# lambdaclass/simpleworks

Hardware: AMD Instinct MI355X
Metric: Marlin prove() constraints/sec at 2^20 R1CS; G1 MSM points/sec (higher is better)
Workload: dtype u32 limbs (384-bit Montgomery Fq for G1, 256-bit Fr); 1 GPU; marlin_prove: synthetic R1CS, 2^20 constraints = variables = non-zeros per matrix (|H| = |K| = 2^20), SRS + proving key device resident; per_gpu_units=1048576, multi_gpu=replicas (one proof per rank)

## Files before the change

simpleworks_amd/_lib.py:

```python
import ctypes
import json
import os

import numpy as np

_HERE = os.path.dirname(os.path.abspath(__file__))
LIB_PATH = os.environ.get("SWM_LIB_PATH") or os.path.join(_HERE, "libswmarlin.so")

_u64p = ctypes.POINTER(ctypes.c_uint64)
_u32p = ctypes.POINTER(ctypes.c_uint32)
_vp = ctypes.c_void_p
_sz = ctypes.c_size_t
_int = ctypes.c_int

ABI = {
    "swm_version": (_int, []),
    "swm_strerror": (ctypes.c_char_p, [_int]),
    "swm_init": (_int, [_int, ctypes.POINTER(_vp)]),
    "swm_destroy": (None, [_vp]),
    "swm_last_error": (ctypes.c_char_p, [_vp]),
    "swm_set_stream": (_int, [_vp, _vp]),
    "swm_set_msm_sharding": (_int, [_vp, ctypes.c_uint, ctypes.c_uint, _vp, _vp]),
    "swm_rccl_unique_id": (_int, [ctypes.c_void_p]),
    "swm_rccl_init": (_int, [_vp, ctypes.c_void_p, ctypes.c_uint, ctypes.c_uint]),
# ... 415 lines not shown
                    "swm_selftest_g1_codec")
        return out, bad.value

    FR29_OPS = {"mul": 0, "mul_c": 1, "normalize": 2, "cond_sub_2r": 3, "cond_sub_r": 4, "canonical_below_2r": 5,
                "canonical": 6, "sub": 7, "unpack": 8, "pack": 9, "inv": 10, "inv_exact": 11}

    def selftest_fr29(self, op, a9, b9=None, spread9=None):
        a = np.ascontiguousarray(a9, dtype=np.uint32).reshape(-1, 9)
        b = np.ascontiguousarray(b9 if b9 is not None else a, dtype=np.uint32).reshape(-1, 9)
        assert b.shape == a.shape
        sp = np.ascontiguousarray(spread9 if spread9 is not None else np.zeros(9), dtype=np.uint32).reshape(9)
        out = np.zeros_like(a)
        self._check(self.lib.swm_selftest_fr29(self.h, self.FR29_OPS[op], _p32(a), _p32(b), _p32(sp), _p32(out), a.shape[0]),
                    "swm_selftest_fr29")
        return out

    def _poly(self, op, data, n, m, z, pieces, out):
        zz = np.ascontiguousarray(z if z is not None else np.zeros(4), dtype=np.uint64).reshape(4)
        pc = np.ascontiguousarray(pieces if pieces is not None else np.zeros(2), dtype=np.uint64).reshape(-1)
        self._check(self.lib.swm_selftest_poly(self.h, op, data.ctypes.data, n, m, _p64(zz), _p64(pc), pc.size // 2,
                                               out.ctypes.data if out is not None else None), "swm_selftest_poly")

    def selftest_suffix_recurrence(self, a_mont, m, z_mont):
        a = np.ascontiguousarray(a_mont, dtype=np.uint64).reshape(-1, 4).copy()
        self._poly(0, a, a.shape[0], m, z_mont, None, None)
        return a

    def selftest_div_linear(self, p_mont, z_mont):
        p = np.ascontiguousarray(p_mont, dtype=np.uint64).reshape(-1, 4)
        out = np.zeros_like(p)
        self._poly(1, p, p.shape[0], 0, z_mont, None, out)
        return out

    def selftest_poly_eval(self, p_mont, z_mont):
        p = np.ascontiguousarray(p_mont, dtype=np.uint64).reshape(-1, 4)
        out = np.zeros(4, dtype=np.uint64)
        self._poly(2, p, p.shape[0], 0, z_mont, None, out)
        return out

    def selftest_poly_eval_many(self, buf_mont, pieces, z_mont):
        buf = np.ascontiguousarray(buf_mont, dtype=np.uint64).reshape(-1, 4)
        pc = np.asarray(pieces, dtype=np.uint64).reshape(-1, 2)
        out = np.zeros((pc.shape[0], 4), dtype=np.uint64)
        self._poly(3, buf, buf.shape[0], 0, z_mont, pc, out)
        return out

    def selftest_ntt_from(self, src_mont, log_n, inverse=False, coset=False):
        src = np.ascontiguousarray(src_mont, dtype=np.uint64).reshape(-1, 4).copy()
        out = np.zeros((1 << log_n, 4), dtype=np.uint64)
        self._poly(4 + int(bool(inverse)) + 2 * int(bool(coset)), src, src.shape[0], log_n, None, None, out)
        return out, src

    def selftest_ntt_cosets(self, coeffs_mont, log_n, ks):
        src = np.ascontiguousarray(coeffs_mont, dtype=np.uint64).reshape(-1, 4).copy()
        kk = np.ascontiguousarray(ks, dtype=np.uint64).reshape(-1)
        out = np.zeros((kk.size << log_n, 4), dtype=np.uint64)
        self._check(self.lib.swm_selftest_poly(self.h, 9, src.ctypes.data, src.shape[0], log_n, _p64(np.zeros(4, np.uint64)),
                                               _p64(kk), kk.size, out.ctypes.data), "swm_selftest_poly")
        return out.reshape(kk.size, 1 << log_n, 4)

    def selftest_intt_cosets3(self, evals_mont, log_n):
        ev = np.ascontiguousarray(evals_mont, dtype=np.uint64).reshape(-1, 4).copy()
        out = np.zeros_like(ev)
        self._poly(10, ev, ev.shape[0], log_n, None, None, out)
        return out

# ... 17 lines not shown
```

simpleworks_amd/csrc/devops.cuh:

```cuda
#pragma once
#include <chrono>
#include <exception>
#include <functional>
#include <utility>
#include <atomic>
#include "context.h"
#include "ff.cuh"
#include "fill.cuh"
#include "fr29.cuh"
#include "host/chacha.h"
#include "host/marlin_types.h"

namespace swm {

int ntt_run(swm_ctx* ctx, void* d_data, unsigned log_n, int inverse, int coset);
int ntt_run_from(swm_ctx* ctx, void* d_data, unsigned log_n, int inverse, int coset, const void* first_src, size_t src_len);
int ntt_cosets_fwd(swm_ctx* ctx, const void* coeffs, size_t len, unsigned log_n, const unsigned* ks, unsigned ncos, void* out);
int ntt_cosets_inv(swm_ctx* ctx, void* data, unsigned log_n, unsigned ncos);
int ntt_sharded_run(swm_ctx* ctx, void* d_local, unsigned log_n, int inverse, int blocks_in);
struct SpmvPlanHost {
    uint64_t nnz = 0, max_row = 0;
    std::vector<uint32_t> chunks, lrows;
};
struct SpmvPlan {
// ... 202 lines not shown

__device__ __forceinline__ Fr29 fr29_zero() {
    Fr29 r;
#pragma unroll
    for (int i = 0; i < 9; i++) r.l[i] = 0;
    return r;
}
__device__ __forceinline__ Fr29 fr29_below_2r(const Fr29& lazy_below_4r) {
    return fr29_cond_sub(fr29_normalize(lazy_below_4r), Fr29Consts::P2);
}
static __global__ void __launch_bounds__(256) rec_tile_total29(const Fr* __restrict__ a, size_t n, RecConsts rc,
                                                               const Fr* __restrict__ zlow ,
                                                               Fr* __restrict__ totals) {
    SWM_LIGHT_KERNEL();
    __shared__ Fr sm[256];
    const size_t base = (size_t)blockIdx.x * RT_TILE;
    const unsigned t = threadIdx.x;
    const Fr29 z256 = fr29_unpack(rc.z256);
    Fr29 acc = fr29_zero();
#pragma unroll 1
    for (int j = RT_PER - 1; j >= 0; j--) {
        size_t k = base + (size_t)j * 256 + t;
        acc = fr29_mul_fenced(acc, z256);
        if (k < n) acc = fr29_add(acc, fr29_unpack(a[k]));
    }
    sm[t] = fr29_pack(fr29_canonical(fr29_mul_fenced(acc, fr29_unpack(zlow[t])), true));
    __syncthreads();
    for (unsigned s = 128; s > 0; s >>= 1) {
        if (t < s) sm[t] = fp_add(sm[t], sm[t + s]);
        __syncthreads();
    }
    if (t == 0) totals[blockIdx.x] = fp_mul(sm[0], rc.zpow[0]);
}
static __global__ void __launch_bounds__(256) rec_tile_scan29(Fr* __restrict__ a, size_t n, RecConsts rc,
                                                              const Fr* __restrict__ tile_true , size_t ntiles) {
    SWM_LIGHT_KERNEL();
    extern __shared__ __align__(16) unsigned char smem_raw[];
    Fr* tile = reinterpret_cast<Fr*>(smem_raw);
    Fr* hs = tile + RT_TILE + 256;
    const size_t b = blockIdx.x, base = b * RT_TILE;
    const unsigned t = threadIdx.x;
#pragma unroll
    for (int j = 0; j < RT_PER; j++) {
        unsigned e = j * 256 + t;
        size_t k = base + e;
        tile[rt_pad(e)] = k < n ? a[k] : fp_zero<Fr>();
    }
    __syncthreads();
    Fr29 loc[RT_PER];
    {
        const Fr29 z1 = fr29_unpack(rc.zpow[1]);
        Fr29 acc = fr29_zero();
#pragma unroll
        for (int i = RT_PER - 1; i >= 0; i--) {
            acc = fr29_add(fr29_unpack(tile[rt_pad(t * RT_PER + i)]), fr29_mul_fenced(acc, z1));
            loc[i] = acc;
        }
        hs[t] = fr29_pack(fr29_below_2r(acc));
    }
    if (t == 0) hs[256] = b + 1 < ntiles ? tile_true[b + 1] : fp_zero<Fr>();
    __syncthreads();
#pragma unroll 1
    for (int k = 0; k < 9; k++) {
        unsigned d = 1u << k;
        Fr v = hs[t];
        bool has = t + d <= 256;
        Fr o = has ? hs[t + d] : fp_zero<Fr>();
        __syncthreads();
        if (has) hs[t] = fr29_pack(fr29_below_2r(fr29_add(fr29_unpack(v), fr29_mul_fenced(fr29_unpack(o), fr29_unpack(rc.zstep[k])))));
        __syncthreads();
    }
    const Fr29 carry = fr29_unpack(hs[t + 1]);
#pragma unroll
    for (int i = 0; i < RT_PER; i++) {
        const Fr29 v = fr29_add(loc[i], fr29_mul_fenced(carry, fr29_unpack(rc.zpow[RT_PER - i])));
        tile[rt_pad(t * RT_PER + i)] = fr29_pack(fr29_cond_sub(fr29_cond_sub(fr29_cond_sub(fr29_normalize(v), Fr29Consts::P2), Fr29Consts::P2), Fr29Consts::P));
    }
    __syncthreads();
#pragma unroll
    for (int j = 0; j < RT_PER; j++) {
        unsigned e = j * 256 + t;
        size_t k = base + e;
        if (k < n) a[k] = tile[rt_pad(e)];
    }
}

inline void suffix_recurrence(swm_ctx* ctx, Fr* a, size_t n, size_t m, const Fr& z);
inline void suffix_recurrence_tiled(swm_ctx* ctx, Fr* a, size_t n, const Fr& z) {
    size_t ntiles = (n + RT_TILE - 1) / RT_TILE;
    RecConsts rc;
    rc.zpow[0] = fp_one<Fr>();
    for (int i = 1; i <= RT_PER; i++) rc.zpow[i] = fp_mul(rc.zpow[i - 1], z);
    rc.zstep[0] = rc.zpow[RT_PER];
    for (int k = 1; k < 9; k++) rc.zstep[k] = fp_sqr(rc.zstep[k - 1]);
    DVec zlow(ctx, 256), totals(ctx, ntiles);
    rc.z256 = dv_pow256(ctx, z, zlow.p);
    RecConsts rc29;
    const Fr two5 = fp_from_u64<Fr>(32);
    for (int i = 0; i <= RT_PER; i++) rc29.zpow[i] = fp_mul(rc.zpow[i], two5);
    for (int k = 0; k < 9; k++) rc29.zstep[k] = fp_mul(rc.zstep[k], two5);
    rc29.z256 = fp_mul(rc.z256, two5);
    prof_begin(ctx, "rec_tile_total");
    hipLaunchKernelGGL(rec_tile_total29, dim3((unsigned)ntiles), dim3(256), 0, ctx->stream, (const Fr*)a, n, rc29, (const Fr*)zlow.p, totals.p);
    prof_end(ctx);
    hip_check(ctx, hipGetLastError(), "rec_tile_total");
    Fr ztile = rc.z256;
    for (int i = 0; i < 3; i++) ztile = fp_sqr(ztile);
    static_assert(RT_TILE == 2048, "tile exponent");
    suffix_recurrence(ctx, totals.p, ntiles, 1, ztile);
    size_t lds = (size_t)(RT_TILE + 256 + 257) * sizeof(Fr);
    static std::atomic<bool> attr_set[64];
    if (!attr_set[ctx->device & 63].load(std::memory_order_acquire)) {
        hip_check(ctx, hipFuncSetAttribute((const void*)rec_tile_scan29, hipFuncAttributeMaxDynamicSharedMemorySize, (int)lds), "attr");
        attr_set[ctx->device & 63].store(true, std::memory_order_release);
    }
    prof_begin(ctx, "rec_tile_scan");
    hipLaunchKernelGGL(rec_tile_scan29, dim3((unsigned)ntiles), dim3(256), lds, ctx->stream, a, n, rc29, (const Fr*)totals.p, ntiles);
    prof_end(ctx);
    hip_check(ctx, hipGetLastError(), "rec_tile_scan");
}

inline void suffix_recurrence(swm_ctx* ctx, Fr* a, size_t n, size_t m, const Fr& z) {
    if (n == 0) return;
    if (m == 1 && n >= 4 * (size_t)RT_TILE) {
        suffix_recurrence_tiled(ctx, a, n, z);
        return;
    }
    size_t rows = (n + m - 1) / m;
    if (rows <= REC_T) {
        prof_begin(ctx, "rec_serial");
        hipLaunchKernelGGL(rec_serial, dim3((unsigned)((m + 63) / 64)), dim3(64), 0, ctx->stream, a, n, m, z);
        prof_end(ctx);
        hip_check(ctx, hipGetLastError(), "rec_serial");
        return;
    }
    size_t nblk = (rows + REC_T - 1) / REC_T;
    DVec head(ctx, nblk * m);
    unsigned grid = (unsigned)((nblk * m + 255) / 256);
    prof_begin(ctx, "rec_local");
    hipLaunchKernelGGL(rec_local, dim3(grid), dim3(256), 0, ctx->stream, a, n, m, z, head.p, nblk);
    prof_end(ctx);
    hip_check(ctx, hipGetLastError(), "rec_local");
    Fr zt = z;
    for (int i = 0; i < 4; i++) zt = fp_sqr(zt);
    static_assert(REC_T == 16, "zt exponent");
    suffix_recurrence(ctx, head.p, nblk * m, m, zt);
    prof_begin(ctx, "rec_fix");
    hipLaunchKernelGGL(rec_fix, dim3(grid), dim3(256), 0, ctx->stream, a, n, m, z, head.p, nblk);
    prof_end(ctx);
    hip_check(ctx, hipGetLastError(), "rec_fix");
}

struct DivResult {
    DVec work;
};
inline DivResult div_linear(swm_ctx* ctx, const Fr* p, size_t n, const Fr& x, size_t cap = 0) {
    DivResult r;
    r.work = dv_copy_padded(ctx, p, n, std::max<size_t>({n, cap, 1}));
    if (n == 0) r.work.zero();
    suffix_recurrence(ctx, r.work.p, n, 1, x);
    return r;
}

static constexpr int EVAL_PER = 16;
static constexpr int EVAL_TILE = 256 * EVAL_PER;
static __global__ void __launch_bounds__(256) eval_chunks(const Fr* __restrict__ c, size_t n, Fr x256, const Fr* __restrict__ xpow,
                                                          Fr* __restrict__ out) {
    SWM_LIGHT_KERNEL();
    __shared__ Fr sm[256];
    const size_t base = (size_t)blockIdx.x * EVAL_TILE;
    const unsigned t = threadIdx.x;
    Fr acc = fp_zero<Fr>();
#pragma unroll 1
    for (int j = EVAL_PER - 1; j >= 0; j--) {
        size_t k = base + (size_t)j * 256 + t;
        acc = fp_mul(acc, x256);
        if (k < n) acc = fp_add(acc, c[k]);
    }
    sm[t] = fp_mul(acc, xpow[t]);
    __syncthreads();
    for (unsigned s = 128; s > 0; s >>= 1) {
        if (t < s) sm[t] = fp_add(sm[t], sm[t + s]);
        __syncthreads();
    }
    if (t == 0) out[blockIdx.x] = sm[0];
}
struct EvalPoint {
    DVec pw[3];
    Fr y256[3];
};
inline EvalPoint eval_point(swm_ctx* ctx, Fr x) {
    EvalPoint ep;
    for (int l = 0; l < 3; l++) {
        ep.pw[l] = DVec(ctx, 256);
// ... 460 lines not shown
```

simpleworks_amd/csrc/marlin.hip:

```cpp
#include <stdlib.h>
#include <string.h>
#include <algorithm>
#include <chrono>
#include <functional>
#include <memory>
#include "devops.cuh"
#include "g1.cuh"
#include "host/ahp.h"

#include "msm.h"
using namespace swm;

#define LAUNCHX(ctx, name, kernel, grid, block, shmem, ...)                         \
    do {                                                                            \
        prof_begin(ctx, name);                                                      \
        hipLaunchKernelGGL(kernel, grid, block, shmem, (ctx)->stream, __VA_ARGS__); \
        prof_end(ctx);                                                              \
        hip_check(ctx, hipGetLastError(), name);                                    \
    } while (0)

#include "host/pk_codec.h"
#include "host/host_handles.h"
struct swm_srs {
    ~swm_srs() {
// ... 1010 lines not shown
    Fr t = fp_add(fp_add(fp_mul(fp_mul(c.eta_a, x.av[i]), dbc), fp_mul(fp_mul(fp_mul(c.eta_b, x.bv[i]), da), dc)),
                  fp_mul(fp_mul(fp_mul(c.eta_c, x.cv[i]), da), db));
    Fr a_val = fp_mul(c.vhab, t);
    Fr b_val = fp_mul(da, dbc);
    return fp_sub(a_val, fp_mul(b_val, f));
}
struct ProveState {
    ChaChaRng& zk;
    PhaseTrace& tr;
    const ProveShape shape;
    const ShardPlan sp;
    const uint64_t H, K, X, Bsz, M;
    const unsigned logM;
    const size_t nvars, ninst;
    const size_t mask_len;
    const HDomain dh;
    const std::vector<Fr> public_input;
    FiatShamirRng fs;
    VerifierState st;
    Fr rho_w, rho_a, rho_b;
    int lane = 0;
    LPoly P_w, P_za, P_zb, P_mask, P_t, P_g1, P_h1, P_g2, P_h2;
    LPoly idx_polys[12];
    std::map<std::string, LPoly*> polys;
    CommitJob j1[4], j2[3], j3[2];
    std::vector<Commitment> comms1 = std::vector<Commitment>(4), comms2 = std::vector<Commitment>(3),
                            comms3 = std::vector<Commitment>(2);
    bool mask_late = false;
    unsigned mask_pieces = 1;
    AsyncMsm mask_part[2];
    bool ra_closed_form = false;
    bool cosets = false;
    LcSet lcs;
    DVec mask, z, za_evals, zb_evals, za_loc, zb_loc, x_poly, x_evals, w_poly, za_poly, zb_poly, e_za, e_zb, e_z;
    DVec r_alpha_evals, e_ra, t_poly, q1, h1, g1x, f, h2;

    ProveState(const swm_pk& pk, ChaChaRng& rng, PhaseTrace& t, ProveShape shp, const ShardPlan& plan)
        : zk(rng), tr(t), shape(std::move(shp)), sp(plan), H(pk.H), K(pk.K), X(pk.X), Bsz(pk.B), M(4 * pk.H),
          logM(pk.logH + 2), nvars(pk.info.num_variables), ninst(shape.inst.size()), mask_len(3 * pk.H), dh(pk.H),
          public_input(shape.inst.begin() + 1, shape.inst.end()) {
        fs_init(fs, pk.vk, public_input);
        for (int m = 0; m < 3; m++) {
            const DVec* v[4] = {&pk.ar[m].row, &pk.ar[m].col, &pk.ar[m].val, &pk.ar[m].row_col};
            for (int j = 0; j < 4; j++) {
                idx_polys[4 * m + j].p = v[j]->p;
                idx_polys[4 * m + j].n = K;
                polys[kIndexerPolys[4 * m + j]] = &idx_polys[4 * m + j];
            }
        }
        polys["w"] = &P_w; polys["z_a"] = &P_za; polys["z_b"] = &P_zb; polys["mask_poly"] = &P_mask;
        polys["t"] = &P_t; polys["g_1"] = &P_g1; polys["h_1"] = &P_h1; polys["g_2"] = &P_g2; polys["h_2"] = &P_h2;
    }
};

void draw_mask(swm_ctx* ctx, const swm_pk& pk, ProveState& s) {
    const uint64_t H = s.H;
    Fr* mp = s.mask.p;
    if (s.mask_pieces > 1) {
        CommitJob& job = s.j1[3];
        job.has_bound = false;
        job.hiding = false;
        unsigned done_pieces = 0;
        struct PieceEvent {
            hipEvent_t e = nullptr;
            ~PieceEvent() {
                if (e) (void)hipEventDestroy(e);
// ... 466 lines not shown
        });
        rc_check(ctx, ntt_sharded_run(ctx, ab.p, pk.logB, 1, 1));
        DVec loc(ctx, 3 * Kl);
        div_vk(ctx, ab.p, Kl, Bloc, loc.p);
        shard_gather_cyclic(ctx, loc.p, 3 * Kl, s.sp.slog_g, s.h2.p, 3 * K);
    } else if (f_cosets) {
        static const unsigned ks[3] = {1, 2, 3};
        DVec e_f(ctx, 3 * K);
        rc_check(ctx, ntt_cosets_fwd(ctx, s.f.p, K, pk.logK, ks, 3, e_f.p));
        DVec ab(ctx, Bsz);
        Fr* out = ab.p;
        const Fr *pf = e_f.p, *fk = f_K.p;
        const unsigned logK = pk.logK;
        ew(ctx, "round3_pointwise_B", Bsz, [=] __device__(size_t i) {
            const size_t k = i & 3, j = i >> 2;
            out[i] = round3_a_minus_bf(ix, ch, i, k ? pf[((k - 1) << logK) + j] : fk[j]);
        });
        dv_ntt(ctx, ab, pk.logB, true);
        div_vk(ctx, ab.p, K, Bsz, s.h2.p);
    } else {
        DVec e_f = dv_ntt_from(ctx, s.f.p, K, pk.logB, false);
        DVec ab(ctx, Bsz);
        Fr* out = ab.p;
        const Fr* pf = e_f.p;
        ew(ctx, "round3_pointwise_B", Bsz, [=] __device__(size_t i) { out[i] = round3_a_minus_bf(ix, ch, i, pf[i]); });
        dv_ntt(ctx, ab, pk.logB, true);
        div_vk(ctx, ab.p, K, Bsz, s.h2.p);
    }
    s.P_h2.p = s.h2.p;
    s.P_h2.n = 3 * K >= 3 ? 3 * K - 3 : 0;
}

std::vector<Fr> evaluations(swm_ctx* ctx, const swm_pk& pk, ProveState& s) {
    std::map<std::pair<std::string, bool>, Fr> eval_cache;
    {
        std::vector<std::pair<std::string, bool>> want;
        for (const char* l : {"z_b", "t", "g_1", "mask_poly", "z_a", "w", "h_1"}) want.push_back({l, false});
        for (int i = 0; i < 12; i++) want.push_back({kIndexerPolys[i], true});
        want.push_back({"g_2", true});
        want.push_back({"h_2", true});
        DVec slots(ctx, want.size());
        auto enqueue_at = [&](bool at_gamma, const EvalPoint& ep) {
            std::vector<EvalItem> items;
            for (size_t i = 0; i < want.size(); i++) {
                if (want[i].second != at_gamma) continue;
                LPoly* lp = s.polys.at(want[i].first);
                items.push_back({lp->p, lp->n, slots.p + i});
            }
            poly_eval_many(ctx, items, ep);
        };
        EvalPoint ep_beta = eval_point(ctx, s.st.beta);
        enqueue_at(false, ep_beta);
        commit_gather(ctx, {&s.j3[0].plain, &s.j3[0].shifted, &s.j3[1].plain});
        pc_commit_end_round(ctx, pk, {&s.j3[0], &s.j3[1]}, {nullptr, nullptr}, {&s.P_g2.rand, &s.P_h2.rand}, s.comms3.data());
        s.tr.mark("round 3 commitments");
        fs_absorb_commitments(s.fs, s.comms3);
        s.st.gamma = s.fs.rand_fr();
        EvalPoint ep_gamma = eval_point(ctx, s.st.gamma);
        enqueue_at(true, ep_gamma);
        std::vector<Fr> vals = slots.download(0, want.size());
        for (size_t i = 0; i < want.size(); i++) eval_cache[want[i]] = vals[i];
    }
    const Fr beta = s.st.beta, gamma = s.st.gamma;
    auto poly_at = [&](const std::string& label, const Fr& point) {
        bool at_gamma = fp_eq(point, gamma);
        auto key = std::make_pair(label, at_gamma);
        auto it = eval_cache.find(key);
// ... 8 lines not shown
        for (auto& t : terms) acc = fp_add(acc, t.second.empty() ? t.first : fp_mul(t.first, poly_at(t.second, point)));
        return acc;
    };
    s.lcs = construct_linear_combinations(pk.info, s.public_input, provider, s.st);
    std::vector<std::pair<std::string, Fr>> evals;
    for (auto& q : kQuerySet) {
        const Fr& pt = std::string(q.point) == "beta" ? beta : gamma;
        Fr v = provider(q.label, s.lcs.at(q.label), pt);
        if (lc_has_zero_eval(q.label)) {
            if (!fp_is_zero(v) && !ctx->emulated_exchange)
                throw MarlinError(SWM_ERR_UNSATISFIED, std::string(q.label) + " does not evaluate to zero: constraint system is not satisfied");
            continue;
        }
        evals.push_back({q.label, v});
    }
    std::sort(evals.begin(), evals.end(), [](auto& a, auto& b) { return a.first < b.first; });
    std::vector<Fr> out;
    for (auto& e : evals) out.push_back(e.second);
    return out;
}

#ifndef SWM_OPEN_FOLD
#define SWM_OPEN_FOLD 1
#endif
__global__ void __launch_bounds__(256) open_fold_shifted(Fr* __restrict__ wq, const Fr* __restrict__ sq, size_t n, Fr k) {
    SWM_LIGHT_KERNEL();
    for (size_t t = blockIdx.x * (size_t)blockDim.x + threadIdx.x; t < n; t += (size_t)gridDim.x * blockDim.x)
        wq[t] = fp_add(wq[t], fp_mul(sq[t], k));
}
std::vector<PcProof> open_combinations(swm_ctx* ctx, const swm_pk& pk, ProveState& s, const Fr& xi) {
    struct ShiftedTerm {
        LPoly* lp;
        Fr ch;
    };
    static constexpr int MAX_COMBINE = 24;
    struct CombineTerms {
        const Fr* src[MAX_COMBINE];
        size_t len[MAX_COMBINE];
        Fr k[MAX_COMBINE];
    };
    struct PointOpen {
        Fr point;
        DVec comb;
        DivResult wq;
        std::vector<DivResult> sq;
        AsyncMsm wjob;
        std::vector<AsyncMsm> sjobs;
        AsyncMsm folded_slot;
        bool folded = false;
        HPoly r_comb, shifted_r, shifted_r_witness;
        std::vector<ShiftedTerm> shifted_terms;
    };
    const char* points[2] = {"beta", "gamma"};
    PointOpen po[2];
    for (int pi = 0; pi < 2; pi++) {
        const char* pl = points[pi];
        PointOpen& o = po[pi];
        o.point = pi == 0 ? s.st.beta : s.st.gamma;
        const Fr point = o.point;
        std::vector<std::string> labels;
        for (auto& q : kQuerySet)
            if (std::string(q.point) == pl) labels.push_back(q.label);
        std::sort(labels.begin(), labels.end());
        size_t plen = 0;
        for (auto& l : labels)
            for (auto& t : s.lcs.at(l))
                if (!t.second.empty()) plen = std::max(plen, s.polys.at(t.second)->n);
        o.comb = DVec(ctx, plen ? plen : 1);
        CombineTerms cterms;
        int nterms = 0;
        Fr ch = fr_one();
        for (auto& l : labels) {
            const LcTerms& terms = s.lcs.at(l);
            bool single_bounded = false;
            for (auto& t : terms) {
                if (t.second.empty()) continue;
                LPoly* lp = s.polys.at(t.second);
                if (terms.size() == 1 && lp->has_bound) single_bounded = true;
                else if (lp->has_bound) throw MarlinError(SWM_ERR_INTERNAL, "EquationHasDegreeBounds");
                Fr k = fp_mul(ch, t.first);
                if (nterms >= MAX_COMBINE) throw MarlinError(SWM_ERR_INTERNAL, "too many terms in an opening");
                cterms.src[nterms] = lp->p;
                cterms.len[nterms] = lp->n;
                cterms.k[nterms] = k;
                nterms++;
                hp_add_scaled(o.r_comb, lp->rand.rand, k);
            }
            ch = fp_mul(ch, xi);
            if (single_bounded) {
                LPoly* lp = s.polys.at(terms[0].second);
                o.shifted_terms.push_back({lp, ch});
                hp_add_scaled(o.shifted_r, lp->rand.shifted_rand, ch);
                if (!hp_is_zero(lp->rand.shifted_rand)) hp_add_scaled(o.shifted_r_witness, hp_div_linear(lp->rand.shifted_rand, point), ch);
                ch = fp_mul(ch, xi);
            }
        }
        {
            Fr* out = o.comb.p;
            const int nt = nterms;
            ew(ctx, "open_combine", plen, [=] __device__(size_t i) {
                Fr acc = fp_zero<Fr>();
                for (int j = 0; j < nt; j++)
                    if (i < cterms.len[j]) acc = fp_add(acc, fp_mul(cterms.k[j], cterms.src[j][i]));
                out[i] = acc;
            });
        }
        s.tr.tick(pi == 0 ? "open beta: combination enqueued" : "open gamma: combination enqueued");
        size_t wn = plen ? plen - 1 : 0;
        std::vector<bool> folded(o.shifted_terms.size(), false);
        for (size_t i = 0; i < o.shifted_terms.size(); i++) {
            const LPoly* lp = o.shifted_terms[i].lp;
            const size_t off = pk.srs_max_degree - lp->bound, qn = lp->n ? lp->n - 1 : 0;
            folded[i] = SWM_OPEN_FOLD && qn && pk.in_powers(off, qn);
            if (folded[i]) wn = std::max(wn, off + qn);
        }
        o.wq = div_linear(ctx, o.comb.p, plen, point, wn + 1);
        s.tr.tick("  witness quotient enqueued");
        const bool fold_any = std::find(folded.begin(), folded.end(), true) != folded.end();
        if (!fold_any) {
            commit_enqueue(ctx, &s.lane, pk, 0, o.wq.work.p + 1, wn, &o.wjob);
            s.tr.tick("  witness commitment enqueued");
        }
        o.sq.resize(o.shifted_terms.size());
        o.sjobs.reserve(o.shifted_terms.size());
        for (size_t i = 0; i < o.shifted_terms.size(); i++) {
            auto& stt = o.shifted_terms[i];
            o.sq[i] = div_linear(ctx, stt.lp->p, stt.lp->n, point);
            Fr k = stt.ch;
            Fr* q = o.sq[i].work.p;
            const size_t off = pk.srs_max_degree - stt.lp->bound, qn = stt.lp->n ? stt.lp->n - 1 : 0;
            if (folded[i]) {
                const unsigned grid = (unsigned)std::min<size_t>((qn + 255) / 256, 256 * 32);
                LAUNCHX(ctx, "open_fold_shifted", open_fold_shifted, dim3(grid), dim3(256), 0, o.wq.work.p + 1 + off, q + 1, qn, k);
                s.tr.tick("  shifted quotient folded");
                continue;
            }
            ew(ctx, "open_scale", qn, [=] __device__(size_t t) { q[t + 1] = fp_mul(q[t + 1], k); });
            s.tr.tick("  shifted quotient enqueued");
            o.sjobs.emplace_back();
            commit_enqueue(ctx, &s.lane, pk, off, q + 1, qn, &o.sjobs.back());
            s.tr.tick("  shifted commitment enqueued");
        }
        if (fold_any) {
            commit_enqueue(ctx, &s.lane, pk, 0, o.wq.work.p + 1, wn, &o.wjob);
            s.tr.tick("  witness commitment enqueued");
            o.folded = true;
            o.folded_slot.sharded = o.wjob.sharded;
            o.folded_slot.result = g1_xyzz_identity();
// ... 618 lines not shown
        if (n) in.upload((const uint32_t*)data, n);
        const uint32_t total = scan_exclusive_u32(ctx, in.p, res.p, n);
        std::vector<uint32_t> h = res.download(0, n);
        if (n) memcpy(out, h.data(), n * 4);
        ((uint32_t*)out)[n] = total;
        return;
    }
    DVec a(ctx, n);
    if (n) a.upload((const Fr*)data, n);
    if (op == 9) {
        unsigned ks[4];
        for (size_t c = 0; c < npieces; c++) ks[c] = (unsigned)pieces[c];
        DVec t(ctx, npieces << m);
        rc_check(ctx, ntt_cosets_fwd(ctx, a.p, n, (unsigned)m, ks, (unsigned)npieces, t.p));
        std::vector<Fr> h = t.download(0, t.n);
        memcpy(out, h.data(), t.n * sizeof(Fr));
        return;
    }
    if (op == 10) {
        const size_t N = (size_t)1 << m;
        rc_check(ctx, ntt_cosets_inv(ctx, a.p, (unsigned)m, 3));
        DVec t(ctx, 3 * N);
        const Fr* u = a.p;
        Fr* o = t.p;
        const Fr iota = HDomain(4).gen, half = fr_half();
        ew(ctx, "cosets3_solve", N, [=] __device__(size_t j) {
            const Cosets3 c = cosets3_solve(u[j], u[j + N], u[j + 2 * N], iota, half);
            o[j] = c.p0;
            o[j + N] = c.p1;
            o[j + 2 * N] = c.p2;
        });
        std::vector<Fr> h = t.download(0, t.n);
        memcpy(out, h.data(), t.n * sizeof(Fr));
        return;
    }
    if (op == 0) {
        suffix_recurrence(ctx, a.p, n, m, zz);
        std::vector<Fr> h = a.download(0, n);
        if (n) memcpy(data, h.data(), n * sizeof(Fr));
    } else if (op == 1) {
        DivResult r = div_linear(ctx, a.p, n, zz);
        std::vector<Fr> h = r.work.download(0, n);
        if (n) memcpy(out, h.data(), n * sizeof(Fr));
    } else if (op == 2) {
        const Fr v = poly_eval(ctx, a.p, n, zz);
        memcpy(out, v.v, sizeof(Fr));
    } else if (op == 3) {
        for (size_t i = 0; i < npieces; i++)
            if (pieces[2 * i] > n || pieces[2 * i + 1] > n - pieces[2 * i]) throw MarlinError(SWM_ERR_INVALID_ARG, "piece out of range");
        DVec res(ctx, npieces);
        std::vector<EvalItem> items;
        for (size_t i = 0; i < npieces; i++) items.push_back({a.p + pieces[2 * i], (size_t)pieces[2 * i + 1], res.p + i});
        EvalPoint ep = eval_point(ctx, zz);
        poly_eval_many(ctx, items, ep);
        std::vector<Fr> h = res.download(0, npieces);
        if (npieces) memcpy(out, h.data(), npieces * sizeof(Fr));
    } else {
        DVec t = dv_ntt_from(ctx, a.p, n, (unsigned)m, ((op - 4) & 1) != 0, ((op - 4) & 2) != 0);
        std::vector<Fr> h = t.download(0, t.n);
        memcpy(out, h.data(), t.n * sizeof(Fr));
        std::vector<Fr> s = a.download(0, n);
        if (n) memcpy(data, s.data(), n * sizeof(Fr));
    }
}
int swm_selftest_poly(swm_ctx* ctx, int op, void* data, size_t n, size_t m, const uint64_t z[4], const uint64_t* pieces,
                      size_t npieces, void* out) {
    if (!ctx || op < 0 || op > 10 || (n && !data)) return SWM_ERR_INVALID_ARG;
    if ((op >= 1 && op <= 3 && !z) || (op == 0 && (!z || m == 0)) || (op != 0 && !out) || (op == 3 && npieces && !pieces))
        return SWM_ERR_INVALID_ARG;
    if (op >= 4 && op <= 7 && (m < 1 || m > 28 || n > ((size_t)1 << m))) return SWM_ERR_INVALID_ARG;
    if (op == 9) {
        if (m < 1 || m > 26 || n > ((size_t)2 << m) || npieces < 1 || npieces > 4 || !pieces) return SWM_ERR_INVALID_ARG;
        for (size_t c = 0; c < npieces; c++)
            if (pieces[c] > 3) return SWM_ERR_INVALID_ARG;
    }
    if (op == 10 && (m < 1 || m > 26 || n != ((size_t)3 << m))) return SWM_ERR_INVALID_ARG;
    SWM_ON_DEVICE(ctx);
    SWM_GUARD(ctx, selftest_poly_impl(ctx, op, data, n, m, z, pieces, npieces, out));
}
static void selftest_sample_impl(swm_ctx* ctx, ChaChaRng& rng, size_t need, uint64_t* out_mont) {
    DVec d(ctx, need);
    sample_fr_bulk(ctx, rng, d.p, need);
    std::vector<Fr> h = d.download(0, need);
    if (need) memcpy(out_mont, h.data(), need * sizeof(Fr));
}
int swm_selftest_sample_fr(swm_ctx* ctx, swm_rng* rng, size_t need, uint64_t* out_mont) {
    if (!ctx || !rng || (need && !out_mont)) return SWM_ERR_INVALID_ARG;
    SWM_ON_DEVICE(ctx);
    SWM_GUARD(ctx, selftest_sample_impl(ctx, rng->r, need, out_mont));
}

static void selftest_g1_codec_impl(swm_ctx* ctx, int op, const void* in, size_t n, void* out, unsigned* bad) {
    const dim3 grid((unsigned)((n + 255) / 256)), block(256);
    if (op == 0) {
        DBuf<G1Affine> pts(ctx, n);
        DBuf<uint32_t> enc(ctx, n * 24);
        pts.upload((const G1Affine*)in, n);
        LAUNCHX(ctx, "g1_encode_uncompressed", g1_encode_uncompressed_kernel, grid, block, 0, pts.p, n, enc.p);
        std::vector<uint32_t> h = enc.download(0, n * 24);
        memcpy(out, h.data(), n * 96);
// ... 61 lines not shown
```

Before: 22.51 million constraints/s.

## Fuse opening combination, shifted-term fold and tiled division for both points

Adds an open_divide path that combines the opening terms, including the shifted bounded term placed at its SRS offset along with an evaluation correction, directly into the work buffer while computing per-tile totals. Both opening points are handled in one batched launch per stage, using a 2D grid over points. The recursive carry pass over tile totals is replaced by a single-block carry-scan kernel. This is meant to remove the separate combine pass, the per-point division launches and the extra fold step, cutting memory traffic and launch count. In exchange it adds large kernel-argument structs, a gated fused path with a fallback, and a new selftest op.

```diff
diff --git a/simpleworks_amd/_lib.py b/simpleworks_amd/_lib.py
--- a/simpleworks_amd/_lib.py
+++ b/simpleworks_amd/_lib.py
@@ -471,6 +471,25 @@
         self._poly(1, p, p.shape[0], 0, z_mont, None, out)
         return out
 
+    def selftest_open_divide(self, data_mont, points):
+        data = np.ascontiguousarray(data_mont, dtype=np.uint64).reshape(-1, 4)
+        words, sizes = [len(points)], []
+        for pt in points:
+            words += [len(pt["terms"]), pt["cap"], pt["corr_at"], pt["corr"], pt["z"]]
+            length = 0
+            for so, ln, off, k in pt["terms"]:
+                words += [so, ln, off, k]
+                if ln:
+                    length = max(length, off + ln)
+            if any(int(x) for x in data[pt["corr"]]):
+                length = max(length, pt["corr_at"] + 1)
+            sizes.append(max(length, pt["cap"], 1))
+        pc = np.asarray(words, dtype=np.uint64)
+        out = np.zeros((sum(sizes), 4), dtype=np.uint64)
+        self._check(self.lib.swm_selftest_poly(self.h, 11, data.ctypes.data, data.shape[0], out.shape[0], None, _p64(pc), pc.size,
+                                               out.ctypes.data), "swm_selftest_poly")
+        return [out[sum(sizes[:i]):sum(sizes[:i + 1])] for i in range(len(points))]
+
     def selftest_poly_eval(self, p_mont, z_mont):
         p = np.ascontiguousarray(p_mont, dtype=np.uint64).reshape(-1, 4)
         out = np.zeros(4, dtype=np.uint64)
diff --git a/simpleworks_amd/csrc/devops.cuh b/simpleworks_amd/csrc/devops.cuh
--- a/simpleworks_amd/csrc/devops.cuh
+++ b/simpleworks_amd/csrc/devops.cuh
@@ -258,12 +258,29 @@
     }
     if (t == 0) totals[blockIdx.x] = fp_mul(sm[0], rc.zpow[0]);
 }
-static __global__ void __launch_bounds__(256) rec_tile_scan29(Fr* __restrict__ a, size_t n, RecConsts rc,
-                                                              const Fr* __restrict__ tile_true , size_t ntiles) {
+struct RecScanJob {
+    Fr* a;
+    size_t n;
+    const Fr* tile_true;
+    size_t ntiles;
+    RecConsts rc;
+};
+static constexpr int REC_SCAN_JOBS = 2;
+struct RecScanArgs {
+    RecScanJob job[REC_SCAN_JOBS];
+};
+static __global__ void __launch_bounds__(256) rec_tile_scan29(RecScanArgs args) {
     SWM_LIGHT_KERNEL();
     extern __shared__ __align__(16) unsigned char smem_raw[];
     Fr* tile = reinterpret_cast<Fr*>(smem_raw);
     Fr* hs = tile + RT_TILE + 256;
+    const RecScanJob& jb = args.job[blockIdx.y];
+    const size_t ntiles = jb.ntiles;
+    if (blockIdx.x >= ntiles) return;
+    Fr* __restrict__ a = jb.a;
+    const size_t n = jb.n;
+    const Fr* __restrict__ tile_true = jb.tile_true;
+    const RecConsts& rc = jb.rc;
     const size_t b = blockIdx.x, base = b * RT_TILE;
     const unsigned t = threadIdx.x;
 #pragma unroll
@@ -311,29 +328,97 @@
     }
 }
 
-inline void suffix_recurrence(swm_ctx* ctx, Fr* a, size_t n, size_t m, const Fr& z);
-inline void suffix_recurrence_tiled(swm_ctx* ctx, Fr* a, size_t n, const Fr& z) {
-    size_t ntiles = (n + RT_TILE - 1) / RT_TILE;
+struct RecCarryJob {
+    Fr* totals;
+    size_t nt;
+    Fr w;
+    Fr wstep[8];
+};
+struct RecCarryArgs {
+    RecCarryJob job[REC_SCAN_JOBS];
+};
+static __global__ void __launch_bounds__(256) rec_carry_scan(RecCarryArgs args) {
+    SWM_LIGHT_KERNEL();
+    __shared__ Fr hs[256];
+    const RecCarryJob& jb = args.job[blockIdx.x];
+    Fr* __restrict__ T = jb.totals;
+    const size_t nt = jb.nt, L = (nt + 255) / 256;
+    const unsigned t = threadIdx.x;
+    const size_t lo = min((size_t)t * L, nt), hi = min(lo + L, nt);
+    const Fr w = jb.w;
+    Fr acc = fp_zero<Fr>();
+    for (size_t i = hi; i-- > lo;) acc = fp_add(T[i], fp_mul(acc, w));
+    hs[t] = acc;
+    __syncthreads();
+#pragma unroll 1
+    for (int k = 0; k < 8; k++) {
+        const unsigned d = 1u << k;
+        const bool has = t + d < 256;
+        const Fr v = hs[t];
+        const Fr o = has ? hs[t + d] : fp_zero<Fr>();
+        __syncthreads();
+        if (has) hs[t] = fp_add(v, fp_mul(o, jb.wstep[k]));
+        __syncthreads();
+    }
+    acc = t + 1 < 256 ? hs[t + 1] : fp_zero<Fr>();
+    for (size_t i = hi; i-- > lo;) {
+        acc = fp_add(T[i], fp_mul(acc, w));
+        T[i] = acc;
+    }
+}
+
+struct RecPoint {
+    RecConsts rc29;
+    Pow256Args zsq;
+    Fr z256;
+    Fr two5;
+};
+inline RecPoint rec_point(const Fr& z) {
+    RecPoint rp;
     RecConsts rc;
     rc.zpow[0] = fp_one<Fr>();
     for (int i = 1; i <= RT_PER; i++) rc.zpow[i] = fp_mul(rc.zpow[i - 1], z);
     rc.zstep[0] = rc.zpow[RT_PER];
     for (int k = 1; k < 9; k++) rc.zstep[k] = fp_sqr(rc.zstep[k - 1]);
-    DVec zlow(ctx, 256), totals(ctx, ntiles);
-    rc.z256 = dv_pow256(ctx, z, zlow.p);
-    RecConsts rc29;
-    const Fr two5 = fp_from_u64<Fr>(32);
-    for (int i = 0; i <= RT_PER; i++) rc29.zpow[i] = fp_mul(rc.zpow[i], two5);
-    for (int k = 0; k < 9; k++) rc29.zstep[k] = fp_mul(rc.zstep[k], two5);
-    rc29.z256 = fp_mul(rc.z256, two5);
-    prof_begin(ctx, "rec_tile_total");
-    hipLaunchKernelGGL(rec_tile_total29, dim3((unsigned)ntiles), dim3(256), 0, ctx->stream, (const Fr*)a, n, rc29, (const Fr*)zlow.p, totals.p);
+    rp.zsq.sq[0] = z;
+    for (int b = 1; b < 8; b++) rp.zsq.sq[b] = fp_sqr(rp.zsq.sq[b - 1]);
+    rp.z256 = fp_sqr(rp.zsq.sq[7]);
+    rp.two5 = fp_from_u64<Fr>(32);
+    for (int i = 0; i <= RT_PER; i++) rp.rc29.zpow[i] = fp_mul(rc.zpow[i], rp.two5);
+    for (int k = 0; k < 9; k++) rp.rc29.zstep[k] = fp_mul(rc.zstep[k], rp.two5);
+    rp.rc29.z256 = fp_mul(rp.z256, rp.two5);
+    return rp;
+}
+inline RecCarryJob rec_carry_job(const RecPoint& rp, Fr* totals, size_t nt) {
+    RecCarryJob cj;
+    cj.totals = totals;
+    cj.nt = nt;
+    cj.w = rp.z256;
+    for (int i = 0; i < 3; i++) cj.w = fp_sqr(cj.w);
+    static_assert(RT_TILE == 2048, "tile exponent");
+    Fr wl = fp_one<Fr>(), sq = cj.w;
+    for (size_t e = (nt + 255) / 256; e; e >>= 1) {
+        if (e & 1) wl = fp_mul(wl, sq);
+        sq = fp_sqr(sq);
+    }
+    cj.wstep[0] = wl;
+    for (int k = 1; k < 8; k++) cj.wstep[k] = fp_sqr(cj.wstep[k - 1]);
+    return cj;
+}
+inline void rec_carry_and_scan(swm_ctx* ctx, const RecScanJob* jobs, const RecPoint* rps, int njobs) {
+    RecCarryArgs ca;
+    RecScanArgs sa;
+    size_t gx = 0;
+    for (int j = 0; j < REC_SCAN_JOBS; j++) {
+        const int s = j < njobs ? j : 0;
+        sa.job[j] = jobs[s];
+        ca.job[j] = rec_carry_job(rps[s], const_cast<Fr*>(jobs[s].tile_true), jobs[s].ntiles);
+        if (j < njobs) gx = std::max(gx, jobs[j].ntiles);
+    }
+    prof_begin(ctx, "rec_carry_scan");
+    hipLaunchKernelGGL(rec_carry_scan, dim3((unsigned)njobs), dim3(256), 0, ctx->stream, ca);
     prof_end(ctx);
-    hip_check(ctx, hipGetLastError(), "rec_tile_total");
-    Fr ztile = rc.z256;
-    for (int i = 0; i < 3; i++) ztile = fp_sqr(ztile);
-    static_assert(RT_TILE == 2048, "tile exponent");
-    suffix_recurrence(ctx, totals.p, ntiles, 1, ztile);
+    hip_check(ctx, hipGetLastError(), "rec_carry_scan");
     size_t lds = (size_t)(RT_TILE + 256 + 257) * sizeof(Fr);
     static std::atomic<bool> attr_set[64];
     if (!attr_set[ctx->device & 63].load(std::memory_order_acquire)) {
@@ -341,9 +426,22 @@
         attr_set[ctx->device & 63].store(true, std::memory_order_release);
     }
     prof_begin(ctx, "rec_tile_scan");
-    hipLaunchKernelGGL(rec_tile_scan29, dim3((unsigned)ntiles), dim3(256), lds, ctx->stream, a, n, rc29, (const Fr*)totals.p, ntiles);
+    hipLaunchKernelGGL(rec_tile_scan29, dim3((unsigned)gx, (unsigned)njobs), dim3(256), lds, ctx->stream, sa);
     prof_end(ctx);
     hip_check(ctx, hipGetLastError(), "rec_tile_scan");
+}
+
+inline void suffix_recurrence_tiled(swm_ctx* ctx, Fr* a, size_t n, const Fr& z) {
+    size_t ntiles = (n + RT_TILE - 1) / RT_TILE;
+    const RecPoint rp = rec_point(z);
+    DVec zlow(ctx, 256), totals(ctx, ntiles);
+    dv_pow256(ctx, z, zlow.p);
+    prof_begin(ctx, "rec_tile_total");
+    hipLaunchKernelGGL(rec_tile_total29, dim3((unsigned)ntiles), dim3(256), 0, ctx->stream, (const Fr*)a, n, rp.rc29, (const Fr*)zlow.p, totals.p);
+    prof_end(ctx);
+    hip_check(ctx, hipGetLastError(), "rec_tile_total");
+    RecScanJob job{a, n, totals.p, ntiles, rp.rc29};
+    rec_carry_and_scan(ctx, &job, &rp, 1);
 }
 
 inline void suffix_recurrence(swm_ctx* ctx, Fr* a, size_t n, size_t m, const Fr& z) {
@@ -386,6 +484,122 @@
     if (n == 0) r.work.zero();
     suffix_recurrence(ctx, r.work.p, n, 1, x);
     return r;
+}
+
+static constexpr int OPEN_MAX_TERMS = 24;
+struct CombineTerms {
+    const Fr* src[OPEN_MAX_TERMS];
+    size_t len[OPEN_MAX_TERMS];
+    size_t off[OPEN_MAX_TERMS];
+    Fr k[OPEN_MAX_TERMS];
+    int nterms = 0;
+    size_t corr_at = 0;
+    Fr corr;
+    size_t length() const {
+        size_t n = fp_is_zero(corr) ? 0 : corr_at + 1;
+        for (int j = 0; j < nterms; j++)
+            if (len[j]) n = std::max(n, off[j] + len[j]);
+        return n;
+    }
+};
+__device__ __forceinline__ Fr combine_at(const CombineTerms& ct, size_t i) {
+    Fr c = fp_zero<Fr>();
+    for (int j = 0; j < ct.nterms; j++) {
+        const size_t s = i - ct.off[j];
+        if (s < ct.len[j]) c = fp_add(c, fp_mul(ct.k[j], ct.src[j][s]));
+    }
+    if (i == ct.corr_at) c = fp_add(c, ct.corr);
+    return c;
+}
+struct OpenDivJob {
+    CombineTerms terms;
+    Fr* work;
+    size_t cap;
+    Fr* totals;
+    Pow256Args zsq;
+    Fr z256_29, two5;
+};
+struct OpenDivArgs {
+    OpenDivJob job[REC_SCAN_JOBS];
+};
+static_assert(sizeof(OpenDivArgs) <= 4096, "kernel arguments are limited to 4 KB");
+static __global__ void __launch_bounds__(256) open_combine_totals(OpenDivArgs args) {
+    SWM_LIGHT_KERNEL();
+    __shared__ Fr sm[256];
+    const OpenDivJob& jb = args.job[blockIdx.y];
+    const size_t base = (size_t)blockIdx.x * RT_TILE, cap = jb.cap;
+    const unsigned t = threadIdx.x;
+    Fr zt = fp_one<Fr>();
+#pragma unroll
+    for (int b = 0; b < 8; b++)
+        if ((t >> b) & 1) zt = fp_mul(zt, jb.zsq.sq[b]);
+    const Fr29 z256 = fr29_unpack(jb.z256_29);
+    Fr29 acc = fr29_zero();
+#pragma unroll 1
+    for (int j = RT_PER - 1; j >= 0; j--) {
+        const size_t k = base + (size_t)j * 256 + t;
+        acc = fr29_mul_fenced(acc, z256);
+        if (k < cap) {
+            const Fr c = combine_at(jb.terms, k);
+            jb.work[k] = c;
+            acc = fr29_add(acc, fr29_unpack(c));
+        }
+    }
+    sm[t] = fr29_pack(fr29_canonical(fr29_mul_fenced(acc, fr29_unpack(zt)), true));
+    __syncthreads();
+    for (unsigned s = 128; s > 0; s >>= 1) {
+        if (t < s) sm[t] = fp_add(sm[t], sm[t + s]);
+        __syncthreads();
+    }
+    if (t == 0) jb.totals[blockIdx.x] = fp_mul(sm[0], jb.two5);
+}
+struct OpenDivPoint {
+    CombineTerms terms;
+    Fr z;
+    size_t cap = 0;
+};
+inline void open_divide(swm_ctx* ctx, const OpenDivPoint* pts, int npts, DVec* work) {
+    if (npts < 1 || npts > REC_SCAN_JOBS) throw MarlinError(SWM_ERR_INTERNAL, "open_divide: one or two points");
+    size_t n[REC_SCAN_JOBS], cap[REC_SCAN_JOBS], gx = 0;
+    bool tiled = true;
+    for (int p = 0; p < npts; p++) {
+        if (pts[p].terms.nterms < 0 || pts[p].terms.nterms > OPEN_MAX_TERMS) throw MarlinError(SWM_ERR_INTERNAL, "open_divide: too many terms");
+        n[p] = pts[p].terms.length();
+        cap[p] = std::max<size_t>({n[p], pts[p].cap, 1});
+        work[p] = DVec(ctx, cap[p]);
+        tiled = tiled && n[p] >= 4 * (size_t)RT_TILE;
+        gx = std::max(gx, (cap[p] + RT_TILE - 1) / RT_TILE);
+    }
+    if (!tiled) {
+        for (int p = 0; p < npts; p++) {
+            const CombineTerms ct = pts[p].terms;
+            Fr* out = work[p].p;
+            ew(ctx, "open_combine", cap[p], [=] __device__(size_t i) { out[i] = combine_at(ct, i); });
+            suffix_recurrence(ctx, out, n[p], 1, pts[p].z);
+        }
+        return;
+    }
+    DVec totals(ctx, gx * npts);
+    OpenDivArgs da;
+    RecScanJob jobs[REC_SCAN_JOBS];
+    RecPoint rps[REC_SCAN_JOBS];
+    for (int j = 0; j < REC_SCAN_JOBS; j++) {
+        const int p = j < npts ? j : 0;
+        rps[j] = rec_point(pts[p].z);
+        da.job[j].terms = pts[p].terms;
+        da.job[j].work = work[p].p;
+        da.job[j].cap = cap[p];
+        da.job[j].totals = totals.p + (size_t)p * gx;
+        da.job[j].zsq = rps[j].zsq;
+        da.job[j].z256_29 = rps[j].rc29.z256;
+        da.job[j].two5 = rps[j].two5;
+        jobs[j] = RecScanJob{work[p].p, n[p], totals.p + (size_t)p * gx, (n[p] + RT_TILE - 1) / RT_TILE, rps[j].rc29};
+    }
+    prof_begin(ctx, "open_combine_totals");
+    hipLaunchKernelGGL(open_combine_totals, dim3((unsigned)gx, (unsigned)npts), dim3(256), 0, ctx->stream, da);
+    prof_end(ctx);
+    hip_check(ctx, hipGetLastError(), "open_combine_totals");
+    rec_carry_and_scan(ctx, jobs, rps, npts);
 }
 
 static constexpr int EVAL_PER = 16;
diff --git a/simpleworks_amd/csrc/marlin.hip b/simpleworks_amd/csrc/marlin.hip
--- a/simpleworks_amd/csrc/marlin.hip
+++ b/simpleworks_amd/csrc/marlin.hip
@@ -1066,6 +1066,7 @@
     bool ra_closed_form = false;
     bool cosets = false;
     LcSet lcs;
+    std::map<std::pair<std::string, bool>, Fr> eval_cache;
     DVec mask, z, za_evals, zb_evals, za_loc, zb_loc, x_poly, x_evals, w_poly, za_poly, zb_poly, e_za, e_zb, e_z;
     DVec r_alpha_evals, e_ra, t_poly, q1, h1, g1x, f, h2;
 
@@ -1598,7 +1599,7 @@
 }
 
 std::vector<Fr> evaluations(swm_ctx* ctx, const swm_pk& pk, ProveState& s) {
-    std::map<std::pair<std::string, bool>, Fr> eval_cache;
+    std::map<std::pair<std::string, bool>, Fr>& eval_cache = s.eval_cache;
     {
         std::vector<std::pair<std::string, bool>> want;
         for (const char* l : {"z_b", "t", "g_1", "mask_poly", "z_a", "w", "h_1"}) want.push_back({l, false});
@@ -1673,15 +1674,14 @@
     struct ShiftedTerm {
         LPoly* lp;
         Fr ch;
+        std::string label;
     };
-    static constexpr int MAX_COMBINE = 24;
-    struct CombineTerms {
-        const Fr* src[MAX_COMBINE];
-        size_t len[MAX_COMBINE];
-        Fr k[MAX_COMBINE];
-    };
+    static constexpr int MAX_COMBINE = OPEN_MAX_TERMS;
     struct PointOpen {
         Fr point;
+        CombineTerms cterms;
+        size_t plen = 0, wn = 0;
+        std::vector<bool> folded_terms;
         DVec comb;
         DivResult wq;
         std::vector<DivResult> sq;
@@ -1707,8 +1707,9 @@
         for (auto& l : labels)
             for (auto& t : s.lcs.at(l))
                 if (!t.second.empty()) plen = std::max(plen, s.polys.at(t.second)->n);
-        o.comb = DVec(ctx, plen ? plen : 1);
-        CombineTerms cterms;
+        o.plen = plen;
+        CombineTerms& cterms = o.cterms;
+        cterms.corr = fp_zero<Fr>();
         int nterms = 0;
         Fr ch = fr_one();
         for (auto& l : labels) {
@@ -1723,22 +1724,78 @@
                 if (nterms >= MAX_COMBINE) throw MarlinError(SWM_ERR_INTERNAL, "too many terms in an opening");
                 cterms.src[nterms] = lp->p;
                 cterms.len[nterms] = lp->n;
+                cterms.off[nterms] = 0;
                 cterms.k[nterms] = k;
-                nterms++;
+                cterms.nterms = ++nterms;
                 hp_add_scaled(o.r_comb, lp->rand.rand, k);
             }
             ch = fp_mul(ch, xi);
             if (single_bounded) {
                 LPoly* lp = s.polys.at(terms[0].second);
-                o.shifted_terms.push_back({lp, ch});
+                o.shifted_terms.push_back({lp, ch, terms[0].second});
                 hp_add_scaled(o.shifted_r, lp->rand.shifted_rand, ch);
                 if (!hp_is_zero(lp->rand.shifted_rand)) hp_add_scaled(o.shifted_r_witness, hp_div_linear(lp->rand.shifted_rand, point), ch);
                 ch = fp_mul(ch, xi);
             }
         }
+        size_t wn = plen ? plen - 1 : 0;
+        o.folded_terms.assign(o.shifted_terms.size(), false);
+        for (size_t i = 0; i < o.shifted_terms.size(); i++) {
+            const LPoly* lp = o.shifted_terms[i].lp;
+            const size_t off = pk.srs_max_degree - lp->bound, qn = lp->n ? lp->n - 1 : 0;
+            o.folded_terms[i] = SWM_OPEN_FOLD && qn && pk.in_powers(off, qn);
+            if (o.folded_terms[i]) wn = std::max(wn, off + qn);
+        }
+        o.wn = wn;
+    }
+    bool fused = ctx->shard_world <= 1;
+    for (int pi = 0; pi < 2 && fused; pi++) {
+        const PointOpen& o = po[pi];
+        fused = o.plen >= 4 * (size_t)RT_TILE && o.shifted_terms.size() == 1 && o.folded_terms[0] && o.cterms.nterms < MAX_COMBINE &&
+                s.eval_cache.count({o.shifted_terms[0].label, pi == 1}) != 0;
+    }
+    if (fused) {
+        OpenDivPoint dp[2];
+        DVec work[2];
+        for (int pi = 0; pi < 2; pi++) {
+            PointOpen& o = po[pi];
+            const ShiftedTerm& stt = o.shifted_terms[0];
+            CombineTerms& ct = dp[pi].terms;
+            ct = o.cterms;
+            const size_t off = pk.srs_max_degree - stt.lp->bound;
+            ct.src[ct.nterms] = stt.lp->p;
+            ct.len[ct.nterms] = stt.lp->n;
+            ct.off[ct.nterms] = off;
+            ct.k[ct.nterms] = stt.ch;
+            ct.nterms++;
+            ct.corr_at = off;
+            ct.corr = fp_neg(fp_mul(stt.ch, s.eval_cache.at({stt.label, pi == 1})));
+            dp[pi].z = o.point;
+            dp[pi].cap = o.wn + 1;
+        }
+        open_divide(ctx, dp, 2, work);
+        s.tr.tick("open: both merged quotients enqueued");
+        for (int pi = 0; pi < 2; pi++) {
+            PointOpen& o = po[pi];
+            o.wq.work = std::move(work[pi]);
+            commit_enqueue(ctx, &s.lane, pk, 0, o.wq.work.p + 1, o.wn, &o.wjob);
+            s.tr.tick("  witness commitment enqueued");
+            o.folded = true;
+            o.folded_slot.sharded = o.wjob.sharded;
+            o.folded_slot.result = g1_xyzz_identity();
+        }
+    }
+    for (int pi = 0; pi < 2 && !fused; pi++) {
+        PointOpen& o = po[pi];
+        const Fr point = o.point;
+        const size_t plen = o.plen;
+        const CombineTerms cterms = o.cterms;
+        const std::vector<bool>& folded = o.folded_terms;
+        const size_t wn = o.wn;
+        o.comb = DVec(ctx, plen ? plen : 1);
         {
             Fr* out = o.comb.p;
-            const int nt = nterms;
+            const int nt = cterms.nterms;
             ew(ctx, "open_combine", plen, [=] __device__(size_t i) {
                 Fr acc = fp_zero<Fr>();
                 for (int j = 0; j < nt; j++)
@@ -1747,14 +1804,6 @@
             });
         }
         s.tr.tick(pi == 0 ? "open beta: combination enqueued" : "open gamma: combination enqueued");
-        size_t wn = plen ? plen - 1 : 0;
-        std::vector<bool> folded(o.shifted_terms.size(), false);
-        for (size_t i = 0; i < o.shifted_terms.size(); i++) {
-            const LPoly* lp = o.shifted_terms[i].lp;
-            const size_t off = pk.srs_max_degree - lp->bound, qn = lp->n ? lp->n - 1 : 0;
-            folded[i] = SWM_OPEN_FOLD && qn && pk.in_powers(off, qn);
-            if (folded[i]) wn = std::max(wn, off + qn);
-        }
         o.wq = div_linear(ctx, o.comb.p, plen, point, wn + 1);
         s.tr.tick("  witness quotient enqueued");
         const bool fold_any = std::find(folded.begin(), folded.end(), true) != folded.end();
@@ -2439,6 +2488,54 @@
         });
         std::vector<Fr> h = t.download(0, t.n);
         memcpy(out, h.data(), t.n * sizeof(Fr));
+        return;
+    }
+    if (op == 11) {
+        const uint64_t* w = pieces;
+        size_t left = npieces;
+        auto next = [&]() {
+            if (!left) throw MarlinError(SWM_ERR_INVALID_ARG, "open_divide: term list too short");
+            left--;
+            return (size_t)*w++;
+        };
+        auto elem = [&](size_t i) {
+            if (i >= n) throw MarlinError(SWM_ERR_INVALID_ARG, "open_divide: constant out of range");
+            return ((const Fr*)data)[i];
+        };
+        const size_t npts = next();
+        if (npts < 1 || npts > 2) throw MarlinError(SWM_ERR_INVALID_ARG, "open_divide: one or two points");
+        OpenDivPoint dp[2];
+        size_t total = 0;
+        for (size_t p = 0; p < npts; p++) {
+            CombineTerms& ct = dp[p].terms;
+            const size_t nt = next();
+            if (nt > OPEN_MAX_TERMS) throw MarlinError(SWM_ERR_INVALID_ARG, "open_divide: too many terms");
+            dp[p].cap = next();
+            ct.corr_at = next();
+            ct.corr = elem(next());
+            dp[p].z = elem(next());
+            for (size_t j = 0; j < nt; j++) {
+                const size_t so = next(), ln = next();
+                if (so > n || ln > n - so) throw MarlinError(SWM_ERR_INVALID_ARG, "piece out of range");
+                ct.src[j] = a.p + so;
+                ct.len[j] = ln;
+                ct.off[j] = next();
+                ct.k[j] = elem(next());
+                if (ct.off[j] > ((size_t)1 << 40)) throw MarlinError(SWM_ERR_INVALID_ARG, "open_divide: offset out of range");
+            }
+            ct.nterms = (int)nt;
+            if (ct.corr_at > ((size_t)1 << 40) || dp[p].cap > ((size_t)1 << 40)) throw MarlinError(SWM_ERR_INVALID_ARG, "open_divide: out of range");
+            total += std::max<size_t>({ct.length(), dp[p].cap, 1});
+        }
+        if (total != m) throw MarlinError(SWM_ERR_INVALID_ARG, "open_divide: out holds m elements, the points need another count");
+        DVec work[2];
+        open_divide(ctx, dp, (int)npts, work);
+        size_t at = 0;
+        for (size_t p = 0; p < npts; p++) {
+            std::vector<Fr> h = work[p].download(0, work[p].n);
+            memcpy((Fr*)out + at, h.data(), h.size() * sizeof(Fr));
+            at += h.size();
+        }
         return;
     }
     if (op == 0) {
@@ -2472,7 +2569,8 @@
 }
 int swm_selftest_poly(swm_ctx* ctx, int op, void* data, size_t n, size_t m, const uint64_t z[4], const uint64_t* pieces,
                       size_t npieces, void* out) {
-    if (!ctx || op < 0 || op > 10 || (n && !data)) return SWM_ERR_INVALID_ARG;
+    if (!ctx || op < 0 || op > 11 || (n && !data)) return SWM_ERR_INVALID_ARG;
+    if (op == 11 && (!pieces || !npieces || !n)) return SWM_ERR_INVALID_ARG;
     if ((op >= 1 && op <= 3 && !z) || (op == 0 && (!z || m == 0)) || (op != 0 && !out) || (op == 3 && npieces && !pieces))
         return SWM_ERR_INVALID_ARG;
     if (op >= 4 && op <= 7 && (m < 1 || m > 28 || n > ((size_t)1 << m))) return SWM_ERR_INVALID_ARG;
```

Result: no change. 22.71 million constraints/s, median of 6 (+0.9%).
